# soon-yau/upgpt

Measured on AMD Instinct MI355X. Metric: 256x256 images/sec, 50-step DDIM, bs=8/GPU; UNet MFMA util %, higher is better.
Workload: dtype f16; 1 GPU; BASELINE configs[1]: bs=8/GPU, 256x256 px (latent 4x32x32), 50-step DDIM eta=0, text-only cond [B,87,768], UNet(bbox.yaml) + VAE decode, EMA weights, no CFG; batch_per_gpu=8, ddim_steps=50, batches_in_flight_per_gpu=4, lane_hw_queues=measured, parallelism=replica-dp1, one all-gather of images per batch

## Files before the change

### include/upk.h

```cpp
#ifndef UPK_H_
#define UPK_H_

#include <stddef.h>
#include <stdint.h>

#ifdef __cplusplus
extern "C" {
#endif

#define UPK_VERSION 100

#define UPK_OK 0
#define UPK_EINVAL (-1)
#define UPK_ESHAPE (-2)
#define UPK_EWORKSPACE (-3)
#define UPK_EHIP (-4)
#define UPK_ENODEV (-5)

typedef struct upk_ctx upk_ctx;
typedef void* upk_stream;

int upk_version(void);
int upk_create(upk_ctx** out, int device);
int upk_destroy(upk_ctx* ctx);
// ... 169 lines not shown
int upk_gather_rows_f16(upk_ctx* ctx, const void* x, int ldx, const int32_t* idx, int n, int n_src, int dim,
                        void* y, int ldy, upk_stream stream);

int upk_patchify_nchw_f32_f16(upk_ctx* ctx, const float* x, int batch, int c, int h, int w, int patch, void* out,
                              int ld_out, upk_stream stream);
int upk_vit_assemble_f16(upk_ctx* ctx, const void* patch_emb, int ld_patch, const float* class_emb,
                         const float* pos_emb, int batch, int npatch, int dim, void* out, int ld_out,
                         upk_stream stream);

int upk_groupnorm_nhwc_f16(upk_ctx* ctx, const void* x1, int c1, int ld1, const void* x2, int c2,
                           int ld2, int batch, int hw, int groups, const float* gamma,
                           const float* beta, float eps, int fuse_silu, void* y, int ldy,
                           float* stats_ws, upk_stream stream);
size_t upk_groupnorm_ws_bytes(int batch, int hw);
int upk_groupnorm_stats_nhwc_f16(upk_ctx* ctx, const void* x1, int c1, int ld1, const void* x2, int c2, int ld2,
                                 int batch, int hw, int groups, float* stats_ws, upk_stream stream);
int upk_groupnorm_chunks(int hw);
int upk_groupnorm_apply_nhwc_f16(upk_ctx* ctx, const void* x1, int c1, int ld1, const void* x2, int c2,
                                 int ld2, int batch, int hw, int groups, const float* gamma,
                                 const float* beta, float eps, int fuse_silu, void* y, int ldy,
                                 const float* stats_ws, int stats_mode, int stats_nblk, int stats_ld,
                                 const float* stats_ws2, int stats_nblk2, int stats_ld2, upk_stream stream);

int upk_layernorm_f16(upk_ctx* ctx, const void* x, int ldx, int rows, int d, const float* gamma,
                      const float* beta, float eps, void* y, int ldy, upk_stream stream);

int upk_timestep_embed_f16(upk_ctx* ctx, const float* t, int n, int dim, float max_period,
                           void* out, int ld_out, upk_stream stream);

int upk_nchw_f32_to_nhwc_f16(upk_ctx* ctx, const float* x, int batch, int c, int hw, void* y,
                             int ldy, int c_off, int zero_pad_to, float scale,
                             upk_stream stream);
int upk_nhwc_f16_to_nchw_f32(upk_ctx* ctx, const void* x, int ldx, int batch, int c, int hw,
                             float* y, upk_stream stream);
int upk_f32_to_f16(upk_ctx* ctx, const float* x, int rows, int cols, void* y, int ldy,
                   upk_stream stream);

int upk_ddim_step_f32(upk_ctx* ctx, float* x, const float* eps, const float* coefs,
                      const float* noise, const int32_t* step, float* pred_x0, void* xin,
                      int ld_xin, int batch, int c, int hw, upk_stream stream);
int upk_ddim_step_cfg_f32(upk_ctx* ctx, float* x, const float* eps2, const float* coefs,
                          const float* noise, const int32_t* step, float* pred_x0, void* xin,
                          int ld_xin, int batch, int c, int hw, float scale, upk_stream stream);
int upk_ddim_step_edit_f32(upk_ctx* ctx, float* x, const float* eps, const float* coefs, const float* noise,
                           const float* keep, const float* mask, int n_rows, const int32_t* step, float* pred_x0,
                           float* x_plain, void* xin, int ld_xin, int batch, int c, int hw, float scale, int cfg,
// ... 60 lines not shown
```

### upgpt_amd/_lib.py

```python
import contextlib
import ctypes as C
import os
import threading

import torch
from ._check import require

_HERE = os.path.dirname(os.path.abspath(__file__))
LIB_PATH = os.environ.get("UPK_LIB") or os.path.join(_HERE, "libupk.so")

SYMBOLS = [
    "upk_version", "upk_create", "upk_destroy", "upk_last_error", "upk_set_workspace", "upk_num_cus",
    "upk_pack_weight_f16", "upk_packed_weight_bytes", "upk_conv2d_nhwc_f16", "upk_gemm_f16",
    "upk_conv_autotune", "upk_conv_override", "upk_conv_num_configs", "upk_conv_config_name", "upk_conv_gn_fused",
    "upk_conv_ln_rows",
    "upk_geglu_mlp_f16", "upk_geglu_mlp_supported", "upk_cross_block_f16", "upk_cross_block_supported", "upk_head_block_f16", "upk_head_block_supported",
    "upk_attention_f16", "upk_groupnorm_nhwc_f16", "upk_groupnorm_stats_nhwc_f16", "upk_groupnorm_chunks", "upk_groupnorm_apply_nhwc_f16", "upk_groupnorm_finalize_f32", "upk_groupnorm_ws_bytes",
    "upk_layernorm_f16", "upk_timestep_embed_f16",
    "upk_nchw_f32_to_nhwc_f16", "upk_nhwc_f16_to_nchw_f32", "upk_f32_to_f16", "upk_ddim_step_f32",
    "upk_ddim_step_cfg_f32", "upk_ddim_step_edit_f32", "upk_plms_step_f32", "upk_ddpm_step_f32", "upk_attention_causal_f16", "upk_attention_qproj_f16", "upk_embed_tokens_f16",
    "upk_patchify_nchw_f32_f16", "upk_vit_assemble_f16", "upk_gather_rows_f16",
    "upk_image_finish_u8", "upk_ssim_ws_bytes", "upk_ssim_u8",
    "upk_lpips_input_f16", "upk_relu_pool_nhwc_f16", "upk_lpips_ws_bytes", "upk_lpips_layer_f16",
    "upk_advance_step", "upk_step_autoadvance", "upk_kernel_launches", "upk_graph_begin", "upk_graph_end", "upk_graph_launch", "upk_graph_destroy",
    "upk_prof_enable", "upk_prof_collect",
    "upk_stream_create_cumask", "upk_stream_destroy", "upk_probe_placement", "upk_probe_clock",
]

F_SILU, F_GEGLU, F_OUT_F32, F_OUT_NCHW_F32, F_UPSAMPLE2X, F_PAD_ASYM = 0x1, 0x2, 0x4, 0x8, 0x10, 0x20
DDPM_X0, DDPM_CLIP = 0x1, 0x2
LAYOUT_NCHW, LAYOUT_NHWC = 0, 1
FINISH_SAMPLE, FINISH_INPUT, FINISH_DENORM = 0, 1, 2
F_QUICKGELU = 0x40
NUM_CLASSES = 5
CLASS_NAMES = ["igemm", "attention", "groupnorm", "layernorm", "other"]

E_NAMES = {0: "UPK_OK", -1: "UPK_EINVAL", -2: "UPK_ESHAPE", -3: "UPK_EWORKSPACE", -4: "UPK_EHIP", -5: "UPK_ENODEV"}


class UpkError(RuntimeError):
# ... 98 lines not shown
            "upk_cross_block_f16": (C.c_int, [vp, C.POINTER(XblockDesc), vp]),
            "upk_cross_block_supported": (C.c_int, [vp, C.POINTER(XblockDesc)]),
            "upk_head_block_f16": (C.c_int, [vp, C.POINTER(HblockDesc), vp]),
            "upk_head_block_supported": (C.c_int, [vp, C.POINTER(HblockDesc)]),
            "upk_attention_f16": (C.c_int, [vp, vp, i32, i64, vp, i32, i64, vp, i32, vp, i32, i64,
                                            i32, i32, i32, i32, i32, f32, vp]),
            "upk_attention_causal_f16": (C.c_int, [vp, vp, i32, i64, vp, i32, i64, vp, i32, vp, i32, i64,
                                                   i32, i32, i32, i32, f32, vp]),
            "upk_attention_qproj_f16": (C.c_int, [vp, vp, i32, i64, i32, i32, f32, vp, vp, vp, vp, i32, i64, vp, i32, vp,
                                                  i32, i64, i32, i32, i32, i32, i32, f32, vp]),
            "upk_embed_tokens_f16": (C.c_int, [vp, vp, vp, vp, i32, i32, i32, i32, vp, i32, vp]),
            "upk_gather_rows_f16": (C.c_int, [vp, vp, i32, vp, i32, i32, i32, vp, i32, vp]),
            "upk_patchify_nchw_f32_f16": (C.c_int, [vp, vp, i32, i32, i32, i32, i32, vp, i32, vp]),
            "upk_vit_assemble_f16": (C.c_int, [vp, vp, i32, vp, vp, i32, i32, i32, vp, i32, vp]),
            "upk_groupnorm_nhwc_f16": (C.c_int, [vp, vp, i32, i32, vp, i32, i32, i32, i32, i32, vp, vp,
                                                 f32, i32, vp, i32, vp, vp]),
            "upk_groupnorm_stats_nhwc_f16": (C.c_int, [vp, vp, i32, i32, vp, i32, i32, i32, i32, i32, vp, vp]),
            "upk_groupnorm_chunks": (C.c_int, [i32]),
            "upk_groupnorm_apply_nhwc_f16": (C.c_int, [vp, vp, i32, i32, vp, i32, i32, i32, i32, i32, vp, vp,
                                                       f32, i32, vp, i32, vp, i32, i32, i32, vp, i32, i32, vp]),
            "upk_conv_gn_fused": (C.c_int, [vp, C.POINTER(ConvDesc), C.POINTER(C.c_int), C.POINTER(C.c_int)]),
            "upk_groupnorm_finalize_f32": (C.c_int, [vp, vp, i32, i32, i32, i32, i32, i32, vp, vp]),
            "upk_groupnorm_ws_bytes": (C.c_size_t, [i32, i32]),
            "upk_layernorm_f16": (C.c_int, [vp, vp, i32, i32, i32, vp, vp, f32, vp, i32, vp]),
            "upk_timestep_embed_f16": (C.c_int, [vp, vp, i32, i32, f32, vp, i32, vp]),
            "upk_nchw_f32_to_nhwc_f16": (C.c_int, [vp, vp, i32, i32, i32, vp, i32, i32, i32, f32, vp]),
            "upk_nhwc_f16_to_nchw_f32": (C.c_int, [vp, vp, i32, i32, i32, i32, vp, vp]),
            "upk_f32_to_f16": (C.c_int, [vp, vp, i32, i32, vp, i32, vp]),
            "upk_ddim_step_f32": (C.c_int, [vp, vp, vp, vp, vp, vp, vp, vp, i32, i32, i32, i32, vp]),
            "upk_ddim_step_cfg_f32": (C.c_int, [vp, vp, vp, vp, vp, vp, vp, vp, i32, i32, i32, i32, f32, vp]),
            "upk_ddim_step_edit_f32": (C.c_int, [vp, vp, vp, vp, vp, vp, vp, i32, vp, vp, vp, vp, i32, i32, i32, i32, f32,
                                                 i32, vp]),
            "upk_plms_step_f32": (C.c_int, [vp, vp, vp, vp, vp, vp, vp, vp, i32, i32, i32, i32, f32, i32, vp]),
            "upk_ddpm_step_f32": (C.c_int, [vp, vp, vp, vp, vp, vp, vp, vp, vp, vp, vp, i32, i32, i32, i32, i32, vp]),
            "upk_image_finish_u8": (C.c_int, [vp, vp, i32, i32, i32, i32, i64, i32, i32, i32, i32, vp, i64, i32, i64, i32,
                                              C.POINTER(C.c_float), vp]),
            "upk_ssim_ws_bytes": (C.c_size_t, [i32, i32, i32, i32]),
            "upk_ssim_u8": (C.c_int, [vp, vp, i64, i64, vp, i64, i64, i32, i32, i32, i32, vp, vp, C.c_size_t, vp]),
            "upk_lpips_input_f16": (C.c_int, [vp, vp, i32, i64, i64, i32, i32, i32, i32, C.POINTER(C.c_float), vp, i64, vp]),
            "upk_relu_pool_nhwc_f16": (C.c_int, [vp, vp, i32, i32, i32, i32, i32, vp, i32, vp]),
            "upk_lpips_ws_bytes": (C.c_size_t, [i32, i32, i32]),
            "upk_lpips_layer_f16": (C.c_int, [vp, vp, vp, i32, i64, i32, i32, i32, vp, i32, vp, vp, C.c_size_t, vp]),
            "upk_advance_step": (C.c_int, [vp, vp, vp]),
            "upk_step_autoadvance": (C.c_int, [vp, vp]),
            "upk_kernel_launches": (C.c_longlong, [vp, i32]),
            "upk_graph_begin": (C.c_int, [vp, vp]),
# ... 326 lines not shown
```

### upgpt_amd/build.py

```python
import hashlib
import os
import shutil
import subprocess
import sys
from concurrent.futures import ThreadPoolExecutor

HERE = os.path.dirname(os.path.abspath(__file__))
CSRC = os.path.join(HERE, "csrc")
OUT = os.environ.get("UPK_LIB") or os.path.join(HERE, "libupk.so")
SOURCES = ["igemm.hip", "bigtile.hip", "astat.hip", "mlp.hip", "xblock.hip", "attention.hip", "norm.hip", "misc.hip", "image.hip",
           "metrics.hip", "lpips.hip"]
FILE_FLAGS = {"attention.hip": ["-mllvm", "-amdgpu-mfma-vgpr-form", "-fno-honor-nans", "-mno-amdgpu-ieee"],
              "image.hip": ["-ffp-contract=off"], "lpips.hip": ["-ffp-contract=off"]}
ARCH = "gfx950"


def _hipcc():
    for cand in (os.environ.get("HIPCC"), shutil.which("hipcc"), "/opt/rocm/bin/hipcc"):
        if cand and os.path.exists(cand):
            return cand
    raise RuntimeError("hipcc not found: libupk.so cannot be built")


def _source_hash():
    h = hashlib.sha256()
    files = sorted(os.path.join(CSRC, f) for f in os.listdir(CSRC)) + [os.path.join(HERE, "..", "include", "upk.h")]
    for path in files:
        h.update(os.path.basename(path).encode())
        with open(path, "rb") as f:
            h.update(f.read())
    h.update((ARCH + " " + os.environ.get("UPK_CXXFLAGS", "") + repr(sorted(FILE_FLAGS.items()))).encode())
    return h.hexdigest()

# ... 68 lines not shown
```

### upgpt_amd/emitter.py

```python
import ctypes as C
import os

import torch

from . import _lib as L
from . import knobs as K
from ._check import require
from .packing import PW, Packer, _rup, head_pad
from .tuning import TUNE_CACHE, TUNE_CACHE_LANES


class Act:
    __slots__ = ("t", "B", "H", "W", "C", "gn_src", "ln_src")

    def __init__(self, t, B, H, W, C):
        self.t, self.B, self.H, self.W, self.C = t, B, H, W, C
        self.ln_src = None
        self.gn_src = None

    @property
    def ld(self):
        return self.t.shape[-1]

    @property
# ... 180 lines not shown
                fold = e_ln[2] < e_pl[2] + K.LN_LAUNCH_US
        if fold:
            return self.conv(P, x, w[name + "_ln"], flags=flags, ln_eps=1e-5, **kw)
        return self.conv(P, self.layernorm(P, x, *v[norm]), w[name], flags=flags, **kw)

    def conv(self, P, x1, pw, *, x2=None, stride=1, flags=0, residual=None, rowvec=None, rv_bs=0, rv_ss=0,
             step=None, out=None, vt=None, nchw_out=None, out_f32=None, spatial=None, ln_eps=None,
             gn_stats=False, append=None, gn=None, lnr=None, lnr_alt=None):
        B, H, W = spatial if spatial is not None else (x1.B, x1.H, x1.W)
        ks = pw.ksize
        kw_all = dict(stride=stride, flags=flags, residual=residual, rowvec=rowvec, rv_bs=rv_bs, rv_ss=rv_ss, step=step,
                      out=out, vt=vt, nchw_out=nchw_out, out_f32=out_f32, spatial=spatial, ln_eps=ln_eps,
                      gn_stats=gn_stats, append=append, lnr=lnr, lnr_alt=lnr_alt)
        if gn is not None:
            return self.conv(P, self.groupnorm(P, x1, *gn[:5], x2=x2, sole=len(gn) > 5 and gn[5]), pw, **kw_all)
        ups = bool(flags & L.F_UPSAMPLE2X)
        HL, WL = (2 * H, 2 * W) if ups else (H, W)
        if flags & L.F_PAD_ASYM:
            Ho, Wo = (HL + 1 - 3) // 2 + 1, (WL + 1 - 3) // 2 + 1
        else:
            pad = 1 if ks == 3 else 0
            Ho, Wo = (HL + 2 * pad - ks) // stride + 1, (WL + 2 * pad - ks) // stride + 1
        M = B * Ho * Wo
        d = L.ConvDesc()
        d.x1 = x1.t.data_ptr()
        d.c1 = _rup(x1.C, 32)
        d.ld1 = x1.ld
        if x2 is not None:
            d.x2 = x2.t.data_ptr()
            d.c2 = _rup(x2.C, 32)
            d.ld2 = x2.ld
        require(d.c1 + d.c2 == pw.k_packed, lambda: repr(("K mismatch", d.c1, d.c2, pw.k_packed)), ValueError)
        require(d.c1 <= x1.ld and (x2 is None or d.c2 <= x2.ld), "conv: padded channel count exceeds the row stride of its source", ValueError)
        d.batch, d.in_h, d.in_w = B, H, W
        d.ksize, d.stride = ks, stride
        d.w_packed = pw.w.data_ptr()
        d._w_bytes = int(pw.w.numel()) * 2
        d.n_out, d.n_pad = pw.n_out, pw.n_pad
        if pw.bias is not None:
            d.bias = pw.bias.data_ptr()
        phased = K.UPS_PHASES and bool(flags & L.F_UPSAMPLE2X) and pw.w_phase is not None and x2 is None
        if phased:
            d.w_phase = pw.w_phase.data_ptr()
        if residual is not None:
            d.residual = residual.t.data_ptr()
            d.ld_res = residual.ld
# ... 140 lines not shown
                    mode, nblk = C.c_int(0), C.c_int(0)
                    chk(fused_fn(h, C.byref(d), C.byref(mode), C.byref(nblk)))
                    info.append((mode.value if mode.value != 3 or d is mine else 0, nblk.value, d.n_pad, sws.data_ptr()))
                if len(info) == 1 and info[0][0] == 3:
                    return
                if len(info) == 1 and info[0][0] == 2 and info[0][1] > 32:
                    m, nb, ld, p1 = info[0]
                    chk(fin_fn(h, p1, nb, ld, x1.B, x1.H * x1.W, x1.C, 32, ws.data_ptr(), s))
                    chk(apply_fn(h, *a, ws.data_ptr(), 1, 0, 0, None, 0, 0, s))
                    return
                if len(info) == 1 and info[0][0]:
                    m, nb, ld, p1 = info[0]
                    chk(apply_fn(h, *a, p1, m, nb, ld, None, 0, 0, s))
                elif len(info) == 2 and info[0][0] == 2 and info[1][0] == 2 and max(info[0][1], info[1][1]) <= 32:
                    chk(apply_fn(h, *a, info[0][3], 2, info[0][1], info[0][2], info[1][3], info[1][1], info[1][2], s))
                else:
                    chk(fn(h, *a, ws.data_ptr(), s))

            P.add(run, x1, x2, gamma, beta, y, ws, armed, cls="groupnorm",
                  label="gn M%d C%d silu%d" % (x1.M, Cc, int(bool(silu))))
        P.n_launch += 1
        return y

    def layernorm(self, P, x, gamma, beta, eps=1e-5):
        y = Act(self.alloc(x.M, x.C), x.B, x.H, x.W, x.C)
        fn, h, chk = self.lib.upk_layernorm_f16, self.hctx, self._chk
        a = (x.t.data_ptr(), x.ld, x.M, x.C, gamma.data_ptr(), beta.data_ptr(), float(eps), y.t.data_ptr(), y.ld)
        P.add(lambda s: chk(fn(h, *a, s)), x, gamma, beta, y, cls="layernorm", label="ln M%d C%d" % (x.M, x.C))
        return y

    def mlp_rows(self, M):
        if K.MLP_ROWS in (32, 64):
            return K.MLP_ROWS
        return 64 if M // 64 >= self.ctx.num_cus else 32

    def geglu_mlp(self, P, t2, x_in, pw1, pw2, gn_stats=True):
        if K.MLP_FUSE == "0" or t2.C != t2.ld:
            return None
        M, C_ = t2.M, t2.C
        if (K.MLP_FUSE == "auto" and L.concurrency() > 1 and os.environ.get("UPGPT_LANES_TUNING", "1") == "1"
                and M in TUNE_CACHE_LANES.meta.get("__unfuse_mlp_M__", ())):
            return None
        rows = self.mlp_rows(M)
        d = L.MlpDesc()
        d.x, d.ldx, d.m, d.c, d.inner = t2.t.data_ptr(), t2.ld, M, C_, pw1.n_out
        d.w1, d.b1, d.u1 = pw1.w.data_ptr(), pw1.bias.data_ptr(), pw1.ln_colsum.data_ptr()
# ... 146 lines not shown
```

### upgpt_amd/engine.py

```python
import ctypes as C
import os

import torch

from . import _lib as L
from . import knobs as K
from ._check import require
from .arch import UNetArch, VAEArch
from .emitter import Act, Emitter, Program
from .packing import (PW, PackedUNet, PackedVAEDecoder, PackedVAEEncoder, PackedVGG16, Packer, _rup,
                      geglu_rows_map, head_pad, pad_rows_map, qproj_pack, vgg16_convs)
from .tuning import TUNE_CACHE, TuneCache


class UNetPlan(Emitter):

    def __init__(self, ctx, packed: PackedUNet, B, H, W, n_ctx, rows, mode):
        super().__init__(ctx)
        require(mode in ("forward", "sampler"), "UNetPlan mode must be 'forward' or 'sampler'", ValueError)
        self.pk, self.arch = packed, packed.arch
        self.B, self.H, self.W, self.n_ctx, self.rows, self.mode = B, H, W, n_ctx, rows, mode
        a = self.arch
        mc, te = a.model_channels, a.time_embed_dim
        self.cin_pad = _rup(a.in_channels, 32)
# ... 187 lines not shown
        self.ctx.nchw_to_nhwc(x, self.B, x.shape[1], self.H * self.W, self.xin.t, self.xin.ld, c_off, zero_pad_to, 1.0)


class VAEDecodePlan(Emitter):

    def __init__(self, ctx, packed: PackedVAEDecoder, B, h, w, scale_factor):
        super().__init__(ctx)
        self.pk, self.arch = packed, packed.arch
        a = self.arch
        self.B, self.h, self.w = B, h, w
        f = a.factor
        self.z = self.alloc(B, a.embed_dim, h, w, dtype=torch.float32)
        self.img = self.alloc(B, a.out_ch, h * f, w * f, dtype=torch.float32)
        self.gn_ws = self.alloc(max(64, ctx.groupnorm_ws_bytes(B, h * f * w * f) // 4), dtype=torch.float32)
        self.prog = Program(ctx)
        P, W_, V_ = self.prog, packed.w, packed.v
        zin = Act(self.alloc(B * h * w, _rup(a.embed_dim, 32), zero=True), B, h, w, a.embed_dim)
        lib, hh, chk, z = self.lib, self.hctx, self._chk, self.z
        inv = 1.0 / float(scale_factor)
        P.add(lambda s: chk(lib.upk_nchw_f32_to_nhwc_f16(hh, z.data_ptr(), B, a.embed_dim, h * w, zin.t.data_ptr(),
                                                         zin.ld, 0, 0, inv, s)))
        x = self.conv(P, zin, W_["post_quant_conv"],
                      out=Act(self.alloc(B * h * w, _rup(a.z_channels, 32), zero=True), B, h, w, a.z_channels))
        for Lr in a.decoder:
            n = Lr.name
            if Lr.kind == "conv":
                x = self.conv(P, x, W_[n], gn_stats=K.vae_gn_byproduct(x.M))
            elif Lr.kind == "resnet":
                h1 = self.conv(P, x, W_[n + ".conv1"], gn=(*V_[n + ".norm1"], 1e-6, True, self.gn_ws), gn_stats=K.vae_gn_byproduct(x.M))
                sk = self.conv(P, x, W_[n + ".nin_shortcut"]) if Lr.cin != Lr.cout else x
                x = self.conv(P, h1, W_[n + ".conv2"], residual=sk, gn=(*V_[n + ".norm2"], 1e-6, True, self.gn_ws),
                              gn_stats=K.vae_gn_byproduct(x.M))
            elif Lr.kind == "attn":
                c, HW = Lr.ch, x.H * x.W
                xn = self.groupnorm(P, x, *V_[n + ".norm"], 1e-6, False, self.gn_ws)
                qk = Act(self.alloc(x.M, 2 * c), x.B, x.H, x.W, 2 * c)
                vt_ld = _rup(HW, 32)
                vt = self.alloc(x.B, 1, c, vt_ld, zero=True)
                self.conv(P, xn, W_[n + ".qkv"], out=qk,
                          vt=dict(t=vt, heads=1, dhead=c, ld=vt_ld, tokens=HW, **{"from": 2 * c}))
                ao = Act(self.alloc(x.M, c), x.B, x.H, x.W, c)
                self.attention(P, qk.t, 2 * c, HW * 2 * c, qk.t[:, c:], 2 * c, HW * 2 * c, vt, vt_ld, ao.t, c, HW * c,
                               x.B, 1, HW, HW, c, int(c) ** -0.5)
                x = self.conv(P, ao, W_[n + ".proj_out"], residual=x, gn_stats=K.vae_gn_byproduct(x.M))
            elif Lr.kind == "upconv":
                x = self.conv(P, x, W_[n], flags=L.F_UPSAMPLE2X)
            elif Lr.kind == "norm_out":
                x = self.groupnorm(P, x, *V_[n], 1e-6, True, self.gn_ws)
            elif Lr.kind == "conv_out":
                self.conv(P, x, W_[n], nchw_out=self.img)
        self.graph = None

    def run(self, z):
        z = z.to(self.dev, torch.float32).contiguous()
        require(tuple(z.shape) == tuple(self.z.shape), lambda: repr((z.shape, self.z.shape)), ValueError)
        self.z.copy_(z)
        self.prog.run()
        return self.img


class VAEEncodePlan(Emitter):

    def __init__(self, ctx, packed: PackedVAEEncoder, B, H, W):
        super().__init__(ctx)
        self.pk, self.arch = packed, packed.arch
        a = self.arch
        f = a.factor
        require(H % f == 0 and W % f == 0, lambda: "image size must be a multiple of %d" % f, ValueError)
        self.x = self.alloc(B, a.in_channels, H, W, dtype=torch.float32)
        self.moments = self.alloc(B, 2 * a.embed_dim, H // f, W // f, dtype=torch.float32)
        self.gn_ws = self.alloc(max(64, ctx.groupnorm_ws_bytes(B, H * W) // 4), dtype=torch.float32)
        self.prog = Program(ctx)
        P, W_, V_ = self.prog, packed.w, packed.v
        xin = Act(self.alloc(B * H * W, _rup(a.in_channels, 32), zero=True), B, H, W, a.in_channels)
        lib, hh, chk, xs = self.lib, self.hctx, self._chk, self.x
        P.add(lambda s: chk(lib.upk_nchw_f32_to_nhwc_f16(hh, xs.data_ptr(), B, a.in_channels, H * W,
                                                         xin.t.data_ptr(), xin.ld, 0, 0, 1.0, s)))
        x = xin
        for Lr in a.encoder:
            n = Lr.name
            if Lr.kind == "conv":
                x = self.conv(P, x, W_[n], gn_stats=K.vae_gn_byproduct(x.M))
            elif Lr.kind == "resnet":
                h1 = self.conv(P, x, W_[n + ".conv1"], gn=(*V_[n + ".norm1"], 1e-6, True, self.gn_ws), gn_stats=K.vae_gn_byproduct(x.M))
                sk = self.conv(P, x, W_[n + ".nin_shortcut"]) if Lr.cin != Lr.cout else x
                x = self.conv(P, h1, W_[n + ".conv2"], residual=sk, gn=(*V_[n + ".norm2"], 1e-6, True, self.gn_ws),
                              gn_stats=K.vae_gn_byproduct(x.M))
            elif Lr.kind == "attn":
                c, HW = Lr.ch, x.H * x.W
                xn = self.groupnorm(P, x, *V_[n + ".norm"], 1e-6, False, self.gn_ws)
                qk = Act(self.alloc(x.M, 2 * c), x.B, x.H, x.W, 2 * c)
                vt_ld = _rup(HW, 32)
                vt = self.alloc(x.B, 1, c, vt_ld, zero=True)
                self.conv(P, xn, W_[n + ".qkv"], out=qk,
                          vt=dict(t=vt, heads=1, dhead=c, ld=vt_ld, tokens=HW, **{"from": 2 * c}))
                ao = Act(self.alloc(x.M, c), x.B, x.H, x.W, c)
                self.attention(P, qk.t, 2 * c, HW * 2 * c, qk.t[:, c:], 2 * c, HW * 2 * c, vt, vt_ld, ao.t, c, HW * c,
                               x.B, 1, HW, HW, c, int(c) ** -0.5)
                x = self.conv(P, ao, W_[n + ".proj_out"], residual=x)
            elif Lr.kind == "downconv":
                x = self.conv(P, x, W_[n], stride=2, flags=L.F_PAD_ASYM)
            elif Lr.kind == "norm_out":
                x = self.groupnorm(P, x, *V_[n], 1e-6, True, self.gn_ws)
            elif Lr.kind == "conv_out":
                x = self.conv(P, x, W_[n], out=Act(self.alloc(x.M, _rup(Lr.cout, 32), zero=True), x.B, x.H, x.W,
                                                   Lr.cout))
        self.conv(P, x, W_["quant_conv"], nchw_out=self.moments)

    def run(self, img):
        img = img.to(self.dev, torch.float32).contiguous()
# ... 207 lines not shown
```

### upgpt_amd/knobs.py

```python
import os

VAE_GN_BYPRODUCT = os.environ.get("UPGPT_VAE_GN_BYPRODUCT", "0")
VAE_GN_MINM = int(os.environ.get("UPGPT_VAE_GN_MINM", "131072"))


def vae_gn_byproduct(M):
    return VAE_GN_BYPRODUCT == "1" or (VAE_GN_BYPRODUCT == "auto" and M >= VAE_GN_MINM)
UPS_PHASES = os.environ.get("UPGPT_UPS_PHASES", "1") == "1"
LN_ROWS = os.environ.get("UPGPT_LN_ROWS", "1") == "1"
QPROJ_FUSE = os.environ.get("UPGPT_QPROJ_FUSE", "1") == "1"
GN_REDUCE_APPLY = os.environ.get("UPGPT_GN_REDUCE_APPLY", "1") == "1"
MLP_FUSE = os.environ.get("UPGPT_MLP_FUSE", "auto")
MLP_ROWS = int(os.environ.get("UPGPT_MLP_ROWS", "0"))
XBLOCK = os.environ.get("UPGPT_XBLOCK", "auto")
XB_ROWS = int(os.environ.get("UPGPT_XB_ROWS", "0"))
HBLOCK = os.environ.get("UPGPT_HBLOCK", "auto")
HBLOCK_GN = os.environ.get("UPGPT_HBLOCK_GN", "1") == "1"
WEIGHT_PREFETCH = os.environ.get("UPGPT_WEIGHT_PREFETCH", "auto")
WEIGHT_PREFETCH_AHEAD = int(os.environ.get("UPGPT_WEIGHT_PREFETCH_AHEAD", "1"))
WEIGHT_PREFETCH_MAX = int(os.environ.get("UPGPT_WEIGHT_PREFETCH_MAX", str(32 << 20)))
LN_LAUNCH_US = 5.0
```

### upgpt_amd/packing.py

```python
import torch

from . import knobs as K
from ._check import require
from .arch import UNetArch, VAEArch


def _rup(v, m):
    return (v + m - 1) // m * m



def head_pad(d):
    for p in (32, 64, 128, 256, 512):
        if d <= p:
            return p
    raise NotImplementedError("attention head dim %d > 512" % d)


class PW:
    __slots__ = ("w", "n_pad", "bias", "n_out", "k_packed", "ksize", "n_real", "k_real", "ln_colsum", "k_append", "w_phase")


class SharedPacks:

# ... 109 lines not shown
        return p

    def append_1x1(self, main, skip):
        require(skip.ksize == 1 and skip.n_pad == main.n_pad and skip.n_out == main.n_out and main.ln_colsum is None, "append_1x1: the appended weight must be a 1x1 with the main weight's rows", ValueError)
        p = PW()
        p.w = torch.cat([main.w.reshape(-1), skip.w.reshape(-1)])
        p.n_pad, p.n_out, p.ksize, p.k_packed, p.n_real = main.n_pad, main.n_out, main.ksize, main.k_packed, main.n_real
        p.k_append = skip.k_packed
        p.k_real = main.k_real + skip.k_real
        p.ln_colsum = None
        bs = [b for b in (main.bias, skip.bias) if b is not None]
        p.bias = None if not bs else (bs[0] if len(bs) == 1 else bs[0] + bs[1])
        return p

    def pack_product(self, outer, inner):
        wo = self.get(outer + ".weight").float()
        wo = wo.reshape(wo.shape[0], -1)
        wi = self.get(inner + ".weight").float()
        prod = {"p.weight": (wo @ wi).contiguous(), "p.bias": wo @ self.get(inner + ".bias").float()}
        return Packer(self.ctx, lambda n: prod[n]).pack("p")

    def vec(self, name):
        return self.get(name).float().contiguous()


def qproj_pack(w, gamma, beta, heads, dh, dp, cq, dev):
    C_ = w.shape[1]
    wf = torch.zeros(heads, dp, cq, dtype=torch.float32, device=dev)
    wf[:, :dh, :C_] = (w.float().to(dev) * gamma.float().to(dev)[None, :]).reshape(heads, dh, C_)
    bias = torch.zeros(heads, dp, dtype=torch.float32, device=dev)
    bias[:, :dh] = (w.float().to(dev) @ beta.float().to(dev)).reshape(heads, dh)
    w16 = wf.half()
    colsum = w16.float().sum(dim=2)
    r = torch.arange(dp, device=dev)
    kd, t, m = r // 32, (r % 32) // 16, r % 16
    src = 32 * kd + 8 * (m // 4) + 4 * t + (m % 4)
    return w16[:, src, :].contiguous(), colsum.reshape(-1).contiguous(), bias.reshape(-1).contiguous()


def pad_rows_map(parts, heads, dh, dp):
    j = torch.arange(parts * heads * dp)
    part, r = j // (heads * dp), j % (heads * dp)
    h, d = r // dp, r % dp
    return torch.where(d < dh, part * heads * dh + h * dh + d, torch.full_like(j, -1))


# ... 75 lines not shown
            elif Lr.kind == "down":
                w[n + ".op"] = pk.pack(n + ".op")
            elif Lr.kind == "up":
                w[n + ".conv"] = pk.add_upsample_phases(pk.pack(n + ".conv"), n + ".conv")
        norm("out.0")
        w["out.2"] = pk.pack("out.2")
        self.w, self.v = w, v


class PackedVAEDecoder:
    def __init__(self, ctx, arch: VAEArch, get):
        pk = Packer(ctx, get)
        self.arch = arch
        w, v = {}, {}

        def norm(name):
            v[name] = (pk.vec("decoder." + name + ".weight"), pk.vec("decoder." + name + ".bias"))

        w["post_quant_conv"] = pk.pack("post_quant_conv", cin_packed=_rup(arch.embed_dim, 32))
        for Lr in arch.decoder:
            n, d = Lr.name, "decoder." + Lr.name
            if Lr.kind in ("conv", "conv_out"):
                w[n] = pk.pack(d, cin_packed=_rup(Lr.cin, 32))
            elif Lr.kind == "resnet":
                norm(n + ".norm1")
                w[n + ".conv1"] = pk.pack(d + ".conv1")
                norm(n + ".norm2")
                w[n + ".conv2"] = pk.pack(d + ".conv2")
                if Lr.cin != Lr.cout:
                    w[n + ".nin_shortcut"] = pk.pack(d + ".nin_shortcut")
            elif Lr.kind == "attn":
                if Lr.ch not in (32, 64, 128, 256, 512):
                    raise NotImplementedError("VAE AttnBlock width %d" % Lr.ch)
                norm(n + ".norm")
                w[n + ".qkv"] = pk.pack([d + ".q", d + ".k", d + ".v"], n_out=2 * Lr.ch)
                w[n + ".proj_out"] = pk.pack(d + ".proj_out")
            elif Lr.kind == "upconv":
                w[n] = pk.add_upsample_phases(pk.pack(d), d)
            elif Lr.kind == "norm_out":
                norm(n)
        self.w, self.v = w, v


class PackedVAEEncoder:
    def __init__(self, ctx, arch: VAEArch, get):
        pk = Packer(ctx, get)
# ... 62 lines not shown
```

Baseline: 98.36 images/s.

## Fuse VAE decoder norm_out GroupNorm+SiLU into small-N conv_out kernel

Adds a dedicated HIP kernel that applies GroupNorm, SiLU and the final 3x3 conv with at most 4 output channels in one pass. It stages normalized halo tiles in LDS as fp32 and accumulates with scalar FMAs per channel, then reduces across waves and writes NCHW f32 output directly. This removes the separate groupnorm pass and its f16 intermediate, and avoids padding the 3-channel conv to a full MFMA tile. The decoder uses it by default, while the GN stats source is still taken from the byproduct machinery. The trade-off is that the final conv now runs on plain FP32 ALUs instead of matrix cores, and grid size is capped at the CU count.

```diff
diff --git a/include/upk.h b/include/upk.h
--- a/include/upk.h
+++ b/include/upk.h
@@ -215,6 +215,11 @@
                                  const float* stats_ws, int stats_mode, int stats_nblk, int stats_ld,
                                  const float* stats_ws2, int stats_nblk2, int stats_ld2, upk_stream stream);
 
+int upk_gn_silu_conv3x3_small_n(upk_ctx* ctx, const void* x, int ldx, int batch, int h, int w, int c, int groups,
+                                const float* gamma, const float* beta, float eps, const float* stats_ws,
+                                const float* weight, const float* bias, int n_out, float* y, upk_stream stream);
+int upk_gn_silu_conv3x3_small_n_prepare(upk_ctx* ctx, int n_out);
+
 int upk_layernorm_f16(upk_ctx* ctx, const void* x, int ldx, int rows, int d, const float* gamma,
                       const float* beta, float eps, void* y, int ldy, upk_stream stream);
 
diff --git a/upgpt_amd/_lib.py b/upgpt_amd/_lib.py
--- a/upgpt_amd/_lib.py
+++ b/upgpt_amd/_lib.py
@@ -16,6 +16,7 @@
     "upk_conv_ln_rows",
     "upk_geglu_mlp_f16", "upk_geglu_mlp_supported", "upk_cross_block_f16", "upk_cross_block_supported", "upk_head_block_f16", "upk_head_block_supported",
     "upk_attention_f16", "upk_groupnorm_nhwc_f16", "upk_groupnorm_stats_nhwc_f16", "upk_groupnorm_chunks", "upk_groupnorm_apply_nhwc_f16", "upk_groupnorm_finalize_f32", "upk_groupnorm_ws_bytes",
+    "upk_gn_silu_conv3x3_small_n", "upk_gn_silu_conv3x3_small_n_prepare",
     "upk_layernorm_f16", "upk_timestep_embed_f16",
     "upk_nchw_f32_to_nhwc_f16", "upk_nhwc_f16_to_nchw_f32", "upk_f32_to_f16", "upk_ddim_step_f32",
     "upk_ddim_step_cfg_f32", "upk_ddim_step_edit_f32", "upk_plms_step_f32", "upk_ddpm_step_f32", "upk_attention_causal_f16", "upk_attention_qproj_f16", "upk_embed_tokens_f16",
@@ -160,6 +161,9 @@
             "upk_conv_gn_fused": (C.c_int, [vp, C.POINTER(ConvDesc), C.POINTER(C.c_int), C.POINTER(C.c_int)]),
             "upk_groupnorm_finalize_f32": (C.c_int, [vp, vp, i32, i32, i32, i32, i32, i32, vp, vp]),
             "upk_groupnorm_ws_bytes": (C.c_size_t, [i32, i32]),
+            "upk_gn_silu_conv3x3_small_n": (C.c_int, [vp, vp, i32, i32, i32, i32, i32, i32, vp, vp, f32, vp, vp, vp, i32,
+                                                      vp, vp]),
+            "upk_gn_silu_conv3x3_small_n_prepare": (C.c_int, [vp, i32]),
             "upk_layernorm_f16": (C.c_int, [vp, vp, i32, i32, i32, vp, vp, f32, vp, i32, vp]),
             "upk_timestep_embed_f16": (C.c_int, [vp, vp, i32, i32, f32, vp, i32, vp]),
             "upk_nchw_f32_to_nhwc_f16": (C.c_int, [vp, vp, i32, i32, i32, vp, i32, i32, i32, f32, vp]),
diff --git a/upgpt_amd/build.py b/upgpt_amd/build.py
--- a/upgpt_amd/build.py
+++ b/upgpt_amd/build.py
@@ -8,7 +8,7 @@
 HERE = os.path.dirname(os.path.abspath(__file__))
 CSRC = os.path.join(HERE, "csrc")
 OUT = os.environ.get("UPK_LIB") or os.path.join(HERE, "libupk.so")
-SOURCES = ["igemm.hip", "bigtile.hip", "astat.hip", "mlp.hip", "xblock.hip", "attention.hip", "norm.hip", "misc.hip", "image.hip",
+SOURCES = ["igemm.hip", "bigtile.hip", "astat.hip", "mlp.hip", "xblock.hip", "attention.hip", "norm.hip", "gn_conv_out.hip", "misc.hip", "image.hip",
            "metrics.hip", "lpips.hip"]
 FILE_FLAGS = {"attention.hip": ["-mllvm", "-amdgpu-mfma-vgpr-form", "-fno-honor-nans", "-mno-amdgpu-ieee"],
               "image.hip": ["-ffp-contract=off"], "lpips.hip": ["-ffp-contract=off"]}
diff --git a/upgpt_amd/csrc/gn_conv_out.hip b/upgpt_amd/csrc/gn_conv_out.hip
--- /dev/null
+++ b/upgpt_amd/csrc/gn_conv_out.hip
@@ -0,0 +1,296 @@
+#include "common.h"
+
+namespace {
+
+constexpr int GC_TW = 32, GC_TH = 8;
+constexpr int GC_HW = GC_TW + 2, GC_HH = GC_TH + 2;
+constexpr int GC_NPIX = GC_HW * GC_HH;
+constexpr int GC_RS = 40;
+constexpr int GC_PS = GC_HH * GC_RS + 2;
+constexpr int GC_CK = 64;
+constexpr int GC_THREADS = 1024, GC_WAVES = GC_THREADS / 64;
+constexpr int GC_NL = (GC_NPIX * (GC_CK / 8) + GC_THREADS - 1) / GC_THREADS;
+constexpr int GC_WPC = 36;
+constexpr int GC_CMAX = 512;
+
+static_assert(GC_WAVES * 4 * GC_TW * GC_TH <= GC_CK * GC_PS, "the reduction reuses the planes");
+
+typedef const __attribute__((address_space(4))) float gc_cfloat;
+
+struct GcArgs {
+  const f16* x;
+  int ldx, batch, h, w, c;
+  int groups, cpg, nchunks;
+  const float* gamma;
+  const float* beta;
+  float eps;
+  const float* ws;
+  const float* wgt;
+  const float* bias;
+  float* y;
+  int tiles_x, tiles_y;
+};
+
+template <int NOUT>
+__global__ __launch_bounds__(GC_THREADS) void gn_conv_out_kernel(const GcArgs a) {
+  extern __shared__ __attribute__((aligned(16))) float gc_lds[];
+  float* planes = gc_lds;
+  float* scale = gc_lds + GC_CK * GC_PS;
+  float* shift = scale + a.c;
+  float* smean = shift + a.c;
+  float* srstd = smean + UPK_GN_GROUPS_MAX;
+  double* part = (double*)(srstd + UPK_GN_GROUPS_MAX);
+  const int tid = threadIdx.x, lane = tid & 63;
+  const int wave = __builtin_amdgcn_readfirstlane(tid >> 6);
+  const int C = a.c;
+  const int npass = (C + GC_CK - 1) / GC_CK;
+  const int tps = a.tiles_x * a.tiles_y;
+  const long T = (long)a.batch * tps;
+  const int t0 = (int)(T * blockIdx.x / gridDim.x), t1 = (int)(T * (blockIdx.x + 1) / gridDim.x);
+  const int nsteps = (t1 - t0) * npass;
+
+  struct Step {
+    int b, y0, x0, pass, vp;
+  };
+  auto decode = [&](int s) {
+    Step st;
+    const int tile = t0 + s / npass;
+    st.pass = s - (s / npass) * npass;
+    st.b = tile / tps;
+    const int r = tile - st.b * tps;
+    const int ty = r / a.tiles_x;
+    st.y0 = ty * GC_TH;
+    st.x0 = (r - ty * a.tiles_x) * GC_TW;
+    const int left = (C - st.pass * GC_CK) >> 3;
+    st.vp = left < GC_CK / 8 ? left : GC_CK / 8;
+    return st;
+  };
+  auto slot = [&](int k, int& p, int& v) {
+    const int i = tid + k * GC_THREADS;
+    const int q = i >> 1;
+    const int vh = q / GC_NPIX;
+    p = q - vh * GC_NPIX;
+    v = vh * 2 + (i & 1);
+  };
+  f16x8 pre[GC_NL];
+  auto issue = [&](const Step& st) {
+#pragma unroll
+    for (int k = 0; k < GC_NL; ++k) {
+      int p, v;
+      slot(k, p, v);
+      const int row = p / GC_HW, col = p - row * GC_HW;
+      const int gy = st.y0 - 1 + row, gx = st.x0 - 1 + col;
+      const bool ok = v < st.vp && gy >= 0 && gy < a.h && gx >= 0 && gx < a.w;
+      const long pix = (long)st.b * a.h * a.w + (ok ? (long)gy * a.w + gx : 0);
+      pre[k] = *(const f16x8*)(a.x + pix * a.ldx + (ok ? st.pass * GC_CK + v * 8 : 0));
+    }
+  };
+  auto stage = [&](const Step& st) {
+#pragma unroll
+    for (int k = 0; k < GC_NL; ++k) {
+      int p, v;
+      slot(k, p, v);
+      if (v >= st.vp) continue;
+      const int row = p / GC_HW, col = p - row * GC_HW;
+      const int gy = st.y0 - 1 + row, gx = st.x0 - 1 + col;
+      const bool inb = gy >= 0 && gy < a.h && gx >= 0 && gx < a.w;
+      const int ch = st.pass * GC_CK + v * 8;
+      const f32x4 sc0 = *(const f32x4*)(scale + ch), sc1 = *(const f32x4*)(scale + ch + 4);
+      const f32x4 sh0 = *(const f32x4*)(shift + ch), sh1 = *(const f32x4*)(shift + ch + 4);
+      float* dst = planes + (v * 8) * GC_PS + row * GC_RS + col;
+#pragma unroll
+      for (int j = 0; j < 8; ++j) {
+        const float f = (float)pre[k][j] * (j < 4 ? sc0[j] : sc1[j - 4]) + (j < 4 ? sh0[j] : sh1[j - 4]);
+        dst[j * GC_PS] = inb ? upk_silu(f) : 0.f;
+      }
+    }
+  };
+  auto tables = [&](int b) {
+    const int q = tid >> 2, sub = tid & 3;
+    if (q < a.groups * 2) {
+      const float* w = a.ws + (long)b * a.nchunks * a.groups * 2 + q;
+      float v[UPK_GN_MAX_CHUNKS / 4];
+#pragma unroll
+      for (int k = 0; k < UPK_GN_MAX_CHUNKS / 4; ++k) {
+        const int idx = sub + 4 * k;
+        v[k] = w[(long)(idx < a.nchunks ? idx : 0) * a.groups * 2];
+      }
+#pragma unroll
+      for (int k = 0; k < UPK_GN_MAX_CHUNKS / 4; ++k) v[k] = sub + 4 * k < a.nchunks ? v[k] : 0.f;
+      double acc = 0.0;
+#pragma unroll
+      for (int k = 0; k < UPK_GN_MAX_CHUNKS / 4; ++k) acc += (double)v[k];
+      part[tid] = acc;
+    }
+    __syncthreads();
+    if (tid < a.groups) {
+      const double s = ((part[tid * 8 + 0] + part[tid * 8 + 1]) + part[tid * 8 + 2]) + part[tid * 8 + 3];
+      const double ss = ((part[tid * 8 + 4] + part[tid * 8 + 5]) + part[tid * 8 + 6]) + part[tid * 8 + 7];
+      const double n = (double)a.h * a.w * a.cpg;
+      const double mean = s / n;
+      double var = ss / n - mean * mean;
+      if (var < 0.0) var = 0.0;
+      smean[tid] = (float)mean;
+      srstd[tid] = (float)(1.0 / sqrt(var + (double)a.eps));
+    }
+    __syncthreads();
+    for (int ch = tid; ch < C; ch += GC_THREADS) {
+      const int g = ch / a.cpg;
+      const float sc = srstd[g] * a.gamma[ch];
+      scale[ch] = sc;
+      shift[ch] = a.beta[ch] - smean[g] * sc;
+    }
+    __syncthreads();
+  };
+
+  const int cg = lane & 15, lr = ((lane >> 4) & 1) * 2 + (lane >> 5);
+  const int r0 = 2 * lr, c0 = 2 * cg;
+  float acc[4][NOUT];
+#pragma unroll
+  for (int i = 0; i < 4; ++i)
+#pragma unroll
+    for (int n = 0; n < NOUT; ++n) acc[i][n] = 0.f;
+
+  int cur_b = -1;
+  Step st;
+  if (nsteps > 0) {
+    st = decode(0);
+    issue(st);
+  }
+  for (int s = 0; s < nsteps; ++s) {
+    if (st.b != cur_b) {
+      tables(st.b);
+      cur_b = st.b;
+    }
+    stage(st);
+    __syncthreads();
+    Step nx = st;
+    if (s + 1 < nsteps) {
+      nx = decode(s + 1);
+      issue(nx);
+    }
+    const int ckp = st.vp * 8;
+    for (int chl = wave; chl < ckp; chl += GC_WAVES) {
+      const float* pl = planes + chl * GC_PS + r0 * GC_RS + c0;
+      float in[4][4];
+#pragma unroll
+      for (int i = 0; i < 4; ++i) {
+        const f32x2 lo = *(const f32x2*)(pl + i * GC_RS), hi = *(const f32x2*)(pl + i * GC_RS + 2);
+        in[i][0] = lo[0];
+        in[i][1] = lo[1];
+        in[i][2] = hi[0];
+        in[i][3] = hi[1];
+      }
+      gc_cfloat* wc = (gc_cfloat*)(a.wgt + (long)(st.pass * GC_CK + chl) * GC_WPC);
+#pragma unroll
+      for (int ky = 0; ky < 3; ++ky)
+#pragma unroll
+        for (int kx = 0; kx < 3; ++kx)
+#pragma unroll
+          for (int n = 0; n < NOUT; ++n) {
+            const float wv = wc[(ky * 3 + kx) * 4 + n];
+#pragma unroll
+            for (int oy = 0; oy < 2; ++oy)
+#pragma unroll
+              for (int ox = 0; ox < 2; ++ox) acc[oy * 2 + ox][n] = fmaf(in[oy + ky][ox + kx], wv, acc[oy * 2 + ox][n]);
+          }
+    }
+    __syncthreads();
+    if (st.pass == npass - 1) {
+      float* red = planes;
+#pragma unroll
+      for (int n = 0; n < NOUT; ++n)
+#pragma unroll
+        for (int i = 0; i < 4; ++i) {
+          red[(wave * 4 + n) * (GC_TW * GC_TH) + (r0 + (i >> 1)) * GC_TW + c0 + (i & 1)] = acc[i][n];
+          acc[i][n] = 0.f;
+        }
+      __syncthreads();
+      const int n = tid >> 8, px = tid & 255;
+      if (n < NOUT) {
+        float sum = red[n * (GC_TW * GC_TH) + px];
+#pragma unroll
+        for (int w = 1; w < GC_WAVES; ++w) sum += red[(w * 4 + n) * (GC_TW * GC_TH) + px];
+        const int gy = st.y0 + (px >> 5), gx = st.x0 + (px & 31);
+        if (gy < a.h && gx < a.w)
+          a.y[(((long)st.b * NOUT + n) * a.h + gy) * a.w + gx] = sum + (a.bias ? a.bias[n] : 0.f);
+      }
+      __syncthreads();
+    }
+    st = nx;
+  }
+}
+
+template <int NOUT>
+int gc_attr(upk_ctx* ctx) {
+  static unsigned long long mask = 0;
+  return upk_lds_attr_once(ctx, (const void*)gn_conv_out_kernel<NOUT>, &mask);
+}
+
+template <int NOUT>
+int gc_launch(upk_ctx* ctx, const GcArgs& a, int grid, size_t lds, hipStream_t stream) {
+  const int rc = gc_attr<NOUT>(ctx);
+  if (rc) return rc;
+  hipLaunchKernelGGL((gn_conv_out_kernel<NOUT>), dim3(grid), dim3(GC_THREADS), lds, stream, a);
+  return upk_check_launch(ctx, "gn_conv_out");
+}
+
+}
+
+extern "C" int upk_gn_silu_conv3x3_small_n_prepare(upk_ctx* ctx, int n_out) {
+  if (!ctx) return UPK_EINVAL;
+  switch (n_out) {
+    case 1: return gc_attr<1>(ctx);
+    case 2: return gc_attr<2>(ctx);
+    case 3: return gc_attr<3>(ctx);
+    case 4: return gc_attr<4>(ctx);
+    default: return upk_fail(ctx, UPK_ESHAPE, "gn_conv_out: n_out=%d outside 1..4", n_out);
+  }
+}
+
+extern "C" int upk_gn_silu_conv3x3_small_n(upk_ctx* ctx, const void* x, int ldx, int batch, int h, int w, int c, int groups,
+                                           const float* gamma, const float* beta, float eps, const float* stats_ws,
+                                           const float* weight, const float* bias, int n_out, float* y,
+                                           upk_stream stream_) {
+  if (!ctx) return UPK_EINVAL;
+  if (!x || !gamma || !beta || !stats_ws || !weight || !y) return upk_fail(ctx, UPK_EINVAL, "gn_conv_out: null pointer");
+  if (batch <= 0 || h <= 0 || w <= 0) return upk_fail(ctx, UPK_EINVAL, "gn_conv_out: empty");
+  if (c <= 0 || (c & 7) || c > GC_CMAX || (ldx & 7) || ldx < c)
+    return upk_fail(ctx, UPK_ESHAPE, "gn_conv_out: C=%d (ld %d) must be a multiple of 8, <= %d and <= ld", c, ldx, GC_CMAX);
+  if (groups <= 0 || groups > UPK_GN_GROUPS_MAX || c % groups)
+    return upk_fail(ctx, UPK_ESHAPE, "gn_conv_out: C=%d groups=%d unsupported", c, groups);
+  if (n_out < 1 || n_out > 4) return upk_fail(ctx, UPK_ESHAPE, "gn_conv_out: n_out=%d outside 1..4", n_out);
+  if ((long)h * w > (1L << 30) / batch) return upk_fail(ctx, UPK_ESHAPE, "gn_conv_out: more than 2^30 pixels");
+  GcArgs a;
+  a.x = (const f16*)x;
+  a.ldx = ldx;
+  a.batch = batch;
+  a.h = h;
+  a.w = w;
+  a.c = c;
+  a.groups = groups;
+  a.cpg = c / groups;
+  int ppc;
+  upk_gn_chunking(h * w, &a.nchunks, &ppc);
+  a.gamma = gamma;
+  a.beta = beta;
+  a.eps = eps;
+  a.ws = stats_ws;
+  a.wgt = weight;
+  a.bias = bias;
+  a.y = y;
+  a.tiles_x = (w + GC_TW - 1) / GC_TW;
+  a.tiles_y = (h + GC_TH - 1) / GC_TH;
+  const long tiles = (long)batch * a.tiles_x * a.tiles_y;
+  const int grid = (int)(tiles < ctx->num_cus ? tiles : ctx->num_cus);
+  const size_t lds = ((size_t)GC_CK * GC_PS + 2 * (size_t)c + 2 * UPK_GN_GROUPS_MAX) * sizeof(float) +
+                     UPK_GN_GROUPS_MAX * 2 * 4 * sizeof(double);
+  hipStream_t stream = (hipStream_t)stream_;
+  upk_prof_scope prof(ctx, UPK_CLS_GN, stream);
+  switch (n_out) {
+    case 1: return gc_launch<1>(ctx, a, grid, lds, stream);
+    case 2: return gc_launch<2>(ctx, a, grid, lds, stream);
+    case 3: return gc_launch<3>(ctx, a, grid, lds, stream);
+    default: return gc_launch<4>(ctx, a, grid, lds, stream);
+  }
+}
diff --git a/upgpt_amd/emitter.py b/upgpt_amd/emitter.py
--- a/upgpt_amd/emitter.py
+++ b/upgpt_amd/emitter.py
@@ -226,6 +226,8 @@
             pad = 1 if ks == 3 else 0
             Ho, Wo = (HL + 2 * pad - ks) // stride + 1, (WL + 2 * pad - ks) // stride + 1
         M = B * Ho * Wo
+        if callable(gn_stats):
+            gn_stats = gn_stats(M)
         d = L.ConvDesc()
         d.x1 = x1.t.data_ptr()
         d.c1 = _rup(x1.C, 32)
@@ -412,6 +414,39 @@
         P.n_launch += 1
         return y
 
+    def gn_silu_conv_small_n(self, P, x, gamma, beta, eps, ws, taps, bias, n_out, nchw_out):
+        fn, h, chk = self.lib.upk_gn_silu_conv3x3_small_n, self.hctx, self._chk
+        stats_fn, fin_fn = self.lib.upk_groupnorm_stats_nhwc_f16, self.lib.upk_groupnorm_finalize_f32
+        fused_fn = self.lib.upk_conv_gn_fused
+        hw = x.H * x.W
+        a = (x.t.data_ptr(), x.ld, x.B, x.H, x.W, x.C, 32, gamma.data_ptr(), beta.data_ptr(), float(eps))
+        b = (taps.data_ptr(), bias.data_ptr(), n_out, nchw_out.data_ptr())
+        armed = self._arm_gn_sources([x])
+        chk(self.lib.upk_gn_silu_conv3x3_small_n_prepare(h, n_out))
+
+        def run(s):
+            stats = ws.data_ptr()
+            mode, nb, ld, sws = 0, 0, 0, None
+            if armed is not None:
+                src, sws = armed[0]
+                if isinstance(src, Emitter.GnProvider):
+                    mode, nb, ld = 2, src.nblk, src.ld
+                else:
+                    m_, n_ = C.c_int(0), C.c_int(0)
+                    chk(fused_fn(h, C.byref(src), C.byref(m_), C.byref(n_)))
+                    mode, nb, ld = m_.value, n_.value, src.n_pad
+            if mode == 1:
+                stats = sws.data_ptr()
+            elif mode == 2:
+                chk(fin_fn(h, sws.data_ptr(), nb, ld, x.B, hw, x.C, 32, ws.data_ptr(), s))
+            else:
+                chk(stats_fn(h, x.t.data_ptr(), x.C, x.ld, None, 0, 0, x.B, hw, 32, ws.data_ptr(), s))
+            chk(fn(h, *a, stats, *b, s))
+
+        P.add(run, x, gamma, beta, ws, taps, bias, nchw_out, armed, cls="groupnorm",
+              label="gn+conv3x3 M%d C%d N%d" % (x.M, x.C, n_out))
+        P.n_launch += 1
+
     def layernorm(self, P, x, gamma, beta, eps=1e-5):
         y = Act(self.alloc(x.M, x.C), x.B, x.H, x.W, x.C)
         fn, h, chk = self.lib.upk_layernorm_f16, self.hctx, self._chk
diff --git a/upgpt_amd/engine.py b/upgpt_amd/engine.py
--- a/upgpt_amd/engine.py
+++ b/upgpt_amd/engine.py
@@ -233,15 +233,16 @@
                                                          zin.ld, 0, 0, inv, s)))
         x = self.conv(P, zin, W_["post_quant_conv"],
                       out=Act(self.alloc(B * h * w, _rup(a.z_channels, 32), zero=True), B, h, w, a.z_channels))
+        fuse_out = False
         for Lr in a.decoder:
             n = Lr.name
             if Lr.kind == "conv":
-                x = self.conv(P, x, W_[n], gn_stats=K.vae_gn_byproduct(x.M))
+                x = self.conv(P, x, W_[n], gn_stats=K.vae_gn_byproduct)
             elif Lr.kind == "resnet":
-                h1 = self.conv(P, x, W_[n + ".conv1"], gn=(*V_[n + ".norm1"], 1e-6, True, self.gn_ws), gn_stats=K.vae_gn_byproduct(x.M))
+                h1 = self.conv(P, x, W_[n + ".conv1"], gn=(*V_[n + ".norm1"], 1e-6, True, self.gn_ws), gn_stats=K.vae_gn_byproduct)
                 sk = self.conv(P, x, W_[n + ".nin_shortcut"]) if Lr.cin != Lr.cout else x
                 x = self.conv(P, h1, W_[n + ".conv2"], residual=sk, gn=(*V_[n + ".norm2"], 1e-6, True, self.gn_ws),
-                              gn_stats=K.vae_gn_byproduct(x.M))
+                              gn_stats=K.vae_gn_byproduct)
             elif Lr.kind == "attn":
                 c, HW = Lr.ch, x.H * x.W
                 xn = self.groupnorm(P, x, *V_[n + ".norm"], 1e-6, False, self.gn_ws)
@@ -253,13 +254,20 @@
                 ao = Act(self.alloc(x.M, c), x.B, x.H, x.W, c)
                 self.attention(P, qk.t, 2 * c, HW * 2 * c, qk.t[:, c:], 2 * c, HW * 2 * c, vt, vt_ld, ao.t, c, HW * c,
                                x.B, 1, HW, HW, c, int(c) ** -0.5)
-                x = self.conv(P, ao, W_[n + ".proj_out"], residual=x, gn_stats=K.vae_gn_byproduct(x.M))
+                x = self.conv(P, ao, W_[n + ".proj_out"], residual=x, gn_stats=K.vae_gn_byproduct)
             elif Lr.kind == "upconv":
                 x = self.conv(P, x, W_[n], flags=L.F_UPSAMPLE2X)
             elif Lr.kind == "norm_out":
-                x = self.groupnorm(P, x, *V_[n], 1e-6, True, self.gn_ws)
+                fuse_out = K.VAE_GN_CONV_OUT and "conv_out.taps" in V_ and x.C == Lr.ch
+                if fuse_out:
+                    norm_out = V_[n]
+                else:
+                    x = self.groupnorm(P, x, *V_[n], 1e-6, True, self.gn_ws)
             elif Lr.kind == "conv_out":
-                self.conv(P, x, W_[n], nchw_out=self.img)
+                if fuse_out:
+                    self.gn_silu_conv_small_n(P, x, *norm_out, 1e-6, self.gn_ws, *V_[n + ".taps"], Lr.cout, self.img)
+                else:
+                    self.conv(P, x, W_[n], nchw_out=self.img)
         self.graph = None
 
     def run(self, z):
@@ -291,12 +299,12 @@
         for Lr in a.encoder:
             n = Lr.name
             if Lr.kind == "conv":
-                x = self.conv(P, x, W_[n], gn_stats=K.vae_gn_byproduct(x.M))
+                x = self.conv(P, x, W_[n], gn_stats=K.vae_gn_byproduct)
             elif Lr.kind == "resnet":
-                h1 = self.conv(P, x, W_[n + ".conv1"], gn=(*V_[n + ".norm1"], 1e-6, True, self.gn_ws), gn_stats=K.vae_gn_byproduct(x.M))
+                h1 = self.conv(P, x, W_[n + ".conv1"], gn=(*V_[n + ".norm1"], 1e-6, True, self.gn_ws), gn_stats=K.vae_gn_byproduct)
                 sk = self.conv(P, x, W_[n + ".nin_shortcut"]) if Lr.cin != Lr.cout else x
                 x = self.conv(P, h1, W_[n + ".conv2"], residual=sk, gn=(*V_[n + ".norm2"], 1e-6, True, self.gn_ws),
-                              gn_stats=K.vae_gn_byproduct(x.M))
+                              gn_stats=K.vae_gn_byproduct)
             elif Lr.kind == "attn":
                 c, HW = Lr.ch, x.H * x.W
                 xn = self.groupnorm(P, x, *V_[n + ".norm"], 1e-6, False, self.gn_ws)
diff --git a/upgpt_amd/knobs.py b/upgpt_amd/knobs.py
--- a/upgpt_amd/knobs.py
+++ b/upgpt_amd/knobs.py
@@ -6,6 +6,7 @@
 
 def vae_gn_byproduct(M):
     return VAE_GN_BYPRODUCT == "1" or (VAE_GN_BYPRODUCT == "auto" and M >= VAE_GN_MINM)
+VAE_GN_CONV_OUT = os.environ.get("UPGPT_VAE_GN_CONV_OUT", "1") == "1"
 UPS_PHASES = os.environ.get("UPGPT_UPS_PHASES", "1") == "1"
 LN_ROWS = os.environ.get("UPGPT_LN_ROWS", "1") == "1"
 QPROJ_FUSE = os.environ.get("UPGPT_QPROJ_FUSE", "1") == "1"
diff --git a/upgpt_amd/packing.py b/upgpt_amd/packing.py
--- a/upgpt_amd/packing.py
+++ b/upgpt_amd/packing.py
@@ -155,6 +155,13 @@
 
     def vec(self, name):
         return self.get(name).float().contiguous()
+
+    def taps_small_n(self, name):
+        w = self.get(name + ".weight").float().to(self.dev)
+        require(w.dim() == 4 and tuple(w.shape[2:]) == (3, 3) and w.shape[0] <= 4, "taps_small_n: a 3x3 conv weight with <= 4 outputs", ValueError)
+        t = torch.zeros(w.shape[1], 3, 3, 4, dtype=torch.float32, device=self.dev)
+        t[..., : w.shape[0]] = w.half().float().permute(1, 2, 3, 0)
+        return t.contiguous(), self.get(name + ".bias").float().to(self.dev).contiguous()
 
 
 def qproj_pack(w, gamma, beta, heads, dh, dp, cq, dev):
@@ -276,6 +283,8 @@
             n, d = Lr.name, "decoder." + Lr.name
             if Lr.kind in ("conv", "conv_out"):
                 w[n] = pk.pack(d, cin_packed=_rup(Lr.cin, 32))
+                if Lr.kind == "conv_out" and Lr.cout <= 4 and Lr.cin % 8 == 0 and Lr.cin <= 512:
+                    v[n + ".taps"] = pk.taps_small_n(d)
             elif Lr.kind == "resnet":
                 norm(n + ".norm1")
                 w[n + ".conv1"] = pk.pack(d + ".conv1")
```

Result: no change. 97.87 images/s (-0.5%).
